# heyblackC/DFMIR

Measured on AMD Instinct MI355X. Metric: train-step image-pairs/sec (fwd+bwd): 2D 256x256 bs=16 and 3D 160^3 bs=1, higher is better.
Workload: dtype f32 (fp16x2-split MFMA, fp32 accumulate)

## Files before the change

### dfmir_amd/_lib.py

```python
import ctypes
import os
from ctypes import c_float, c_int, c_longlong, c_void_p, POINTER, Structure

_HERE = os.path.dirname(os.path.abspath(__file__))
LIB_PATH = os.environ.get("DFMIR_HIP_LIB") or os.path.join(_HERE, "libdfmir_hip.so")


class DfConvGeom(Structure):
    _fields_ = [(n, c_int) for n in (
        "N", "Cin", "Cout", "Di", "Hi", "Wi", "Do", "Ho", "Wo", "KD", "KH", "KW",
        "stride", "dil", "pd", "ph", "pw", "pad_mode", "act")] + [("slope", c_float)]


P = c_void_p
_GP = POINTER(DfConvGeom)
_SIGS = {
    "dfmir_abi_version": [],
    "dfmir_set_option": [ctypes.c_char_p, ctypes.c_char_p],
    "dfmir_get_option": [ctypes.c_char_p, ctypes.c_char_p, c_int],
    "dfmir_conv_fwd": [_GP, P, P, P, P, P],
    "dfmir_conv_wgrad": [_GP, P, P, P, P],
    "dfmir_bias_grad": [P, P, c_int, c_int, c_longlong, P],
    "dfmir_weight_pack": [P, P, c_int, c_int, c_int, c_int, P],
    "dfmir_weight_pack_floats": [c_int, c_int, c_int],
# ... 61 lines not shown
    "dfmir_instnorm_fwd": [P, P, P, P, P, c_int, c_longlong, c_float, c_int, P, P],
    "dfmir_instnorm_stats_ok": [c_longlong],
    "dfmir_instnorm_stats": [P, P, P, c_int, c_longlong, c_float, c_int, P, P],
    "dfmir_instnorm_bwd": [P, P, P, P, P, c_int, c_longlong, c_int, P, P],
    "dfmir_instnorm_bwd_cols_ok": [c_longlong, c_int],
    "dfmir_instnorm_bwd_cols": [P, P, P, P, P, c_int, c_longlong, c_int, P, P, c_int, P],
    "dfmir_in_relu_blurdown_ok": [c_int, c_int],
    "dfmir_in_relu_blurdown_fwd": [P, P, P, P, c_int, c_int, c_int, c_float, P, P],
    "dfmir_in_relu_blurdown_bwd": [P, P, P, P, P, c_int, c_int, c_int, P, P, P],
    "dfmir_act_bwd": [P, P, P, c_longlong, c_int, c_float, P],
    "dfmir_blur_down_fwd": [P, P, c_int, c_int, c_int, P],
    "dfmir_blur_down_bwd": [P, P, c_int, c_int, c_int, P],
    "dfmir_blur_up_fwd": [P, P, c_int, c_int, c_int, P],
    "dfmir_blur_up_bwd": [P, P, c_int, c_int, c_int, P],
    "dfmir_reflect_pad2d_fwd": [P, P, c_int, c_int, c_int, c_int, P],
    "dfmir_reflect_pad2d_bwd": [P, P, c_int, c_int, c_int, c_int, P],
    "dfmir_reflect_pad2d_bwd_add": [P, P, P, c_int, c_int, c_int, c_int, P],
    "dfmir_upcat_fwd": [P, P, P] + [c_int] * 7 + [P],
    "dfmir_upcat_bwd": [P, P, P] + [c_int] * 7 + [P],
    "dfmir_cat_channels_fwd": [P, P, P, c_longlong, c_longlong, c_longlong, P],
    "dfmir_cat_channels_bwd": [P, P, P, c_longlong, c_longlong, c_longlong, P],
    "dfmir_scale": [P, P, c_longlong, c_float, P],
    "dfmir_warp2d_fwd": [P, P, P] + [c_int] * 6 + [P],
    "dfmir_warp2d_bwd": [P, P, P, P, P] + [c_int] * 6 + [P],
    "dfmir_warp3d_fwd": [P, P, P] + [c_int] * 7 + [P],
    "dfmir_warp3d_bwd": [P, P, P, P, P] + [c_int] * 7 + [P],
    "dfmir_warp_bwd_own_ws_floats": [c_int] * 6,
    "dfmir_warp_bwd_own": [c_int, P, P, P, P, P] + [c_int] * 7 + [P, P],
    "dfmir_resize_fwd": [P, P] + [c_int] * 7 + [c_float, P],
    "dfmir_resize_bwd": [P, P] + [c_int] * 7 + [c_float, P],
    "dfmir_resize_bwd_ws_floats": [c_int] * 7,
    "dfmir_resize_bwd_sep": [P, P] + [c_int] * 7 + [c_float, P, P],
    "dfmir_patch_gather_fwd": [P, P, P, c_int, c_int, c_longlong, c_int, P],
    "dfmir_patch_gather_bwd": [P, P, P, c_int, c_int, c_longlong, c_int, P],
    "dfmir_patch_gather_bwd_amax": [P, P, P, c_int, c_int, c_longlong, c_int, P, P],
    "dfmir_patch_gather_fwd_g": [P, P, P, c_int, c_int, c_longlong, c_int, c_int, P],
    "dfmir_patch_gather_bwd_g": [P, P, P, c_int, c_int, c_longlong, c_int, c_int, P, P],
    "dfmir_l2norm_fwd": [P, P, P, c_int, c_longlong, c_float, P],
    "dfmir_l2norm_bwd": [P, P, P, P, c_int, c_longlong, c_float, P],
    "dfmir_patchnce_fwd": [P, P, P, P, c_longlong, c_int, c_int, c_float, P],
    "dfmir_patchnce_bwd": [P, P, P, P, c_longlong, c_int, c_int, c_float, P],
    "dfmir_masked_l1_fwd": [P, P, P, c_float, P, P, c_longlong, P],
    "dfmir_masked_l1_bwd": [P, P, P, c_float, P, P, P, P, c_longlong, P],
    "dfmir_flow_smooth_ws_floats": [],
    "dfmir_flow_smooth_fwd": [P, P, P] + [c_int] * 5 + [P],
    "dfmir_flow_smooth_bwd": [P, P, P] + [c_int] * 5 + [P],
    "dfmir_flow_smooth_fwd_p": [P, P, P] + [c_int] * 6 + [P],
    "dfmir_flow_smooth_bwd_p": [P, P, P] + [c_int] * 6 + [P],
    "dfmir_mul": [P, P, P, c_longlong, P],
    "dfmir_bend_ws_floats": [c_int] * 5,
    "dfmir_bend_fwd": [P, P, P] + [c_int] * 5 + [c_float] * 3 + [P],
    "dfmir_bend_bwd": [P, P, P] + [c_int] * 5 + [c_float] * 3 + [P],
    "dfmir_invcons_ws_floats": [c_int] * 5,
    "dfmir_invcons_fwd": [c_int, P, P, P, P, P, P] + [c_int] * 4 + [P],
    "dfmir_invcons_bwd_ws_floats": [c_int] * 5,
    "dfmir_invcons_bwd": [c_int, P, P, P, P, P, P, P] + [c_int] * 4 + [P],
    "dfmir_nmi_ws_floats": [c_longlong, c_int],
    "dfmir_nmi_fwd": [P, P, P, P, c_int, c_float, c_float, c_longlong, P, P, P],
    "dfmir_nmi_bwd": [P, P, P, P, c_int, c_float, c_float, c_longlong, P, P, P, P, P],
    "dfmir_mind_ws_floats": [c_int] * 8,
    "dfmir_mind_desc": [P] + [c_int] * 7 + [P, P, P],
    "dfmir_mind_fwd": [P, P, P] + [c_int] * 7 + [P, P, P],
    "dfmir_mind_bwd": [P, P, P] + [c_int] * 7 + [P, P, P, P, P, P],
    "dfmir_warp_dice_ws_floats": [c_int] * 6,
    "dfmir_warp_dice_fwd": [c_int, P, P, P, P] + [c_int] * 6 + [P, P, P, P, P],
    "dfmir_warp_dice_bwd": [c_int, P, P, P, P] + [c_int] * 5 + [P, P, P, P],
    "dfmir_label_hausdorff_ws_bytes": [c_int] * 6,
    "dfmir_label_edt_sq": [c_int, P, c_int, c_int] + [c_int] * 4 + [P, P],
    "dfmir_label_hausdorff": [c_int, P, P, P] + [c_int] * 7 + [P, P, P, P, P, P],
    "dfmir_dice_ws_floats": [c_longlong, c_longlong],
    "dfmir_dice_fwd": [P, P, c_longlong, c_longlong, P, P, P],
    "dfmir_dice_bwd": [P, P, c_longlong, c_longlong, P, P, P, P, P],
    "dfmir_mse_ws_floats": [c_longlong],
    "dfmir_mse_fwd": [P, P, c_longlong, P, P, P],
    "dfmir_mse_bwd": [P, P, c_longlong, P, P, P, P],
    "dfmir_ncc_fwd_m": [P, P, P, c_int, P, P, P, P] + [c_int] * 5 + [c_float, P],
    "dfmir_ncc_bwd_m": [P, P, P, c_int, P, P, P, P, P, P] + [c_int] * 5 + [c_float, P],
    "dfmir_ncc_gauss_fwd": [P, P, P, c_int, P, P, P, P] + [c_int] * 4 + [P, c_int, c_float, c_float, P],
    "dfmir_ncc_gauss_bwd": [P, P, P, c_int, P, P, P, P, P, P] + [c_int] * 4 + [P, c_int, c_float, c_float, P],
    "dfmir_ncc_fwd": [P, P, P, P, P, P] + [c_int] * 5 + [c_float, P],
    "dfmir_ncc_bwd": [P, P, P, P, P, P, P, P] + [c_int] * 5 + [c_float, P],
    "dfmir_patch_gather_fwd_multi": [P, c_int, P, P, c_int, c_int, c_longlong, c_int, P],
    "dfmir_nce_head_fwd": [P, c_int, P, P, P, P, P, P, P, P, P, P, c_int, c_int, c_longlong, c_int, c_float, P],
    "dfmir_patch_ids_draw": [P, P, c_int, c_int, c_int, P, P],
    "dfmir_segment_means_fwd": [P, P, c_int, c_int, c_longlong, c_float, P],
    "dfmir_segment_means_bwd": [P, P, c_int, c_int, c_longlong, c_float, P],
    "dfmir_scalar_combine_fwd": [P, c_int, P, c_int, P, P],
    "dfmir_scalar_combine_bwd": [P, c_int, P, c_int, P, P],
    "dfmir_det_head_floats": [],
    "dfmir_det_begin": [P, c_longlong, P, c_longlong, P, c_int, P, c_longlong, P, c_int, ctypes.c_double, P],
    "dfmir_det_end": [P, P, c_longlong, P, c_longlong, P],
    "dfmir_fill_zero": [P, c_longlong, P],
    "dfmir_sum_scaled": [P, P, c_longlong, c_float, P],
    "dfmir_fill_from_scalar": [P, P, c_longlong, c_float, P],
    "dfmir_adam_step": [P, P, P, P, c_longlong] + [c_float] * 7 + [P],
}

_lib = None


class DfmirHipError(RuntimeError):
    pass


def lib():
    global _lib
    if _lib is None:
        import torch
        if not os.path.exists(LIB_PATH):
            raise DfmirHipError(
                "libdfmir_hip.so not found at %s -- build it with `python -c 'import __graft_entry__ as g; "
                "g.build()'` or `make -C dfmir_amd/csrc` (there is no CPU fallback)" % LIB_PATH)
        h = ctypes.CDLL(LIB_PATH)
        for name, args in _SIGS.items():
            fn = getattr(h, name)
            fn.argtypes = args
            fn.restype = c_int
        h.dfmir_weight_pack_floats.restype = c_longlong
        h.dfmir_conv3d_split_ws_floats.restype = c_longlong
        h.dfmir_conv3d_up_ws_floats.restype = c_longlong
        h.dfmir_conv3d_up_dgrad_ws_floats.restype = c_longlong
        h.dfmir_conv3d_upwgrad_ws_floats.restype = c_longlong
        h.dfmir_flow_smooth_ws_floats.restype = c_longlong
        h.dfmir_bend_ws_floats.restype = c_longlong
        h.dfmir_invcons_ws_floats.restype = c_longlong
        h.dfmir_invcons_bwd_ws_floats.restype = c_longlong
        h.dfmir_nmi_ws_floats.restype = c_longlong
        h.dfmir_mind_ws_floats.restype = c_longlong
        h.dfmir_warp_dice_ws_floats.restype = c_longlong
        h.dfmir_label_hausdorff_ws_bytes.restype = c_longlong
        h.dfmir_dice_ws_floats.restype = c_longlong
        h.dfmir_mse_ws_floats.restype = c_longlong
        h.dfmir_warp_bwd_own_ws_floats.restype = c_longlong
        h.dfmir_resize_bwd_ws_floats.restype = c_longlong
        h.dfmir_last_error.argtypes = []
        h.dfmir_last_error.restype = ctypes.c_char_p
        _lib = h
    return _lib


def check(rc):
    if rc != 0:
        msg = lib().dfmir_last_error()
        raise DfmirHipError(msg.decode() if msg else "dfmir_hip error %d" % rc)


def set_option(name, value=None):
    check(lib().dfmir_set_option(name.encode(), None if value is None else str(value).encode()))


def get_option(name):
    buf = ctypes.create_string_buffer(256)
    n = lib().dfmir_get_option(name.encode(), buf, 256)
    return None if n < 0 else buf.value.decode()


def exported_symbols():
    return sorted(list(_SIGS.keys()) + ["dfmir_last_error"])
```

### dfmir_amd/csrc/nce_head.hip

```cpp
#include "common.h"

#define DF_IDS_MAXP 1024
#define DF_IDS_MAXPERM 4096
struct DfIdSizes {
  long long S[8];
};

__device__ __forceinline__ unsigned long long df_mix64(unsigned long long z) {
  z += 0x9E3779B97F4A7C15ull;
  z = (z ^ (z >> 30)) * 0xBF58476D1CE4E5B9ull;
  z = (z ^ (z >> 27)) * 0x94D049BB133111EBull;
  return z ^ (z >> 31);
}

__global__ __launch_bounds__(256) void patch_ids_draw_k(unsigned long long* __restrict__ state, DfIdSizes sizes,
                                                        int n_layers, int n_sets, int P, int Ppad,
                                                        long long* __restrict__ out) {
  __shared__ unsigned long long el[DF_IDS_MAXPERM];
  __shared__ unsigned char lost[DF_IDS_MAXP];
  __shared__ int pending;
  const int layer = blockIdx.x / n_sets, set = blockIdx.x - layer * n_sets;
  const unsigned long long S = (unsigned long long)sizes.S[layer];
  const unsigned long long seed = state[0], counter = state[1];
  const unsigned long long stream = df_mix64(seed ^ df_mix64(counter * 0x100000001B3ull + (unsigned long long)blockIdx.x));
// ... 203 lines not shown
    _Pragma("unroll") for (int u = 0; u < NH_KB; ++u) {                                           \
      const int kr = 2 * u + hi;                                                                  \
      const bool ok = kr < (KTOT_);                                                               \
      ca0[u] = ok ? wp[(long long)kr * NH_M] : 0.f;                                               \
      ca1[u] = ok ? wp[(long long)kr * NH_M + 32] : 0.f;                                          \
    }                                                                                             \
    for (int j = 0; j < nb; ++j) {                                                                \
      if (j + 1 < nb) {                                                                           \
        _Pragma("unroll") for (int u = 0; u < NH_KB; ++u) {                                       \
          const int kr = 2 * ((j + 1) * NH_KB + u) + hi;                                          \
          const bool ok = kr < (KTOT_);                                                           \
          na0[u] = ok ? wp[(long long)kr * NH_M] : 0.f;                                           \
          na1[u] = ok ? wp[(long long)kr * NH_M + 32] : 0.f;                                      \
        }                                                                                         \
      }                                                                                           \
      _Pragma("unroll") for (int u = 0; u < NH_KB; ++u) {                                         \
        const int kr = 2 * (j * NH_KB + u) + hi;                                                  \
        const float bv = (SRC_)[kr * NH_R + l31];                                                 \
        acc[0] = __builtin_amdgcn_mfma_f32_32x32x2f32(ca0[u], bv, acc[0], 0, 0, 0);               \
        acc[1] = __builtin_amdgcn_mfma_f32_32x32x2f32(ca1[u], bv, acc[1], 0, 0, 0);               \
      }                                                                                           \
      _Pragma("unroll") for (int u = 0; u < NH_KB; ++u) { ca0[u] = na0[u]; ca1[u] = na1[u]; }     \
    }                                                                                             \
  }
  NH_GEMM(k.w1, k.C, Xs)
#pragma unroll
  for (int i = 0; i < 2; ++i)
#pragma unroll
    for (int e = 0; e < 16; ++e) {
      const int m = m0 + 32 * i + (e >> 2) * 8 + hi * 4 + (e & 3);
      float v = acc[i][e] + k.b1[m];
      v = v > 0.f ? v : 0.f;
      Hs[m * NH_R + l31] = v;
      if (k.hs && r0 + l31 < k.rows) k.hs[(long long)m * k.rows + r0 + l31] = v;
      acc[i][e] = 0.f;
    }
  __syncthreads();
  NH_GEMM(k.w2, NH_M, Hs)
#undef NH_GEMM
  float ss = 0.f;
#pragma unroll
  for (int i = 0; i < 2; ++i)
#pragma unroll
    for (int e = 0; e < 16; ++e) {
      const int m = m0 + 32 * i + (e >> 2) * 8 + hi * 4 + (e & 3);
      acc[i][e] += k.b2[m];
      ss += acc[i][e] * acc[i][e];
    }
  ss += __shfl_xor(ss, 32);
  if (hi == 0) red[wid][l31] = ss;
  __syncthreads();
  const float nr = sqrtf((red[0][l31] + red[1][l31]) + (red[2][l31] + red[3][l31]));
  const float inv = 1.f / (nr + k.eps);
  const long long rr = r0 + l31;
  if (rr < k.rows) {
    if (k.nrm && wid == 0 && hi == 0) k.nrm[rr] = nr;
#pragma unroll
    for (int i = 0; i < 2; ++i)
#pragma unroll
      for (int e = 0; e < 16; ++e) {
        const int m = m0 + 32 * i + (e >> 2) * 8 + hi * 4 + (e & 3);
        k.out[(long long)m * k.rows + rr] = acc[i][e] * inv;
        if (k.ypre) k.ypre[(long long)m * k.rows + rr] = acc[i][e];
      }
  }
}
extern "C" int dfmir_nce_head_fwd(const float* const* srcs, int G, const long long* ids, const float* w1, const float* b1,
                                  const float* w2, const float* b2, float* out, float* nrm, float* xs, float* hs,
                                  float* ypre, int Bper, int C, long long S, int P, float eps, void* stream) {
  DF_ARG_CHECK(srcs && ids && w1 && b1 && w2 && b2 && out && G > 0 && G <= 8 && Bper > 0 && C > 0 && C <= NH_CMAX && S > 0 && P > 0);
  NceHeadP k{};
  for (int g = 0; g < G; ++g) {
    DF_ARG_CHECK(srcs[g] != nullptr);
    k.srcs.p[g] = srcs[g];
  }
  k.ids = ids; k.w1 = w1; k.b1 = b1; k.w2 = w2; k.b2 = b2;
  k.out = out; k.nrm = nrm; k.xs = xs; k.hs = hs; k.ypre = ypre;
  k.G = G; k.Bper = Bper; k.C = C; k.P = P; k.S = S; k.rows = (long long)G * Bper * P; k.eps = eps;
  nce_head_fwd_k<<<(unsigned)((k.rows + NH_R - 1) / NH_R), 256, 0, (hipStream_t)stream>>>(k);
  DF_LAUNCH_CHECK();
  return 0;
}

__global__ __launch_bounds__(256) void segment_means_k(const float* __restrict__ rows, float* __restrict__ out, int L,
                                                       int T, long long seg, float scale) {
  __shared__ float sm[17];
  const int t = blockIdx.x;
  float s = 0.f;
  for (int l = 0; l < L; ++l) {
    const float* r = rows + ((long long)l * T + t) * seg;
    for (long long i = threadIdx.x; i < seg; i += 256) s += r[i];
  }
  s = block_sum(s, sm);
  if (threadIdx.x == 0) out[t] = s * (scale / (float)seg);
}
__global__ void segment_means_bwd_k(const float* __restrict__ g, float* __restrict__ drows, int L, int T, long long seg,
                                    float scale) {
  const long long total = (long long)L * T * seg;
  for (long long i = (long long)blockIdx.x * blockDim.x + threadIdx.x; i < total;
       i += (long long)gridDim.x * blockDim.x) {
    const int t = (int)((i / seg) % T);
    drows[i] = g[t] * (scale / (float)seg);
  }
}
extern "C" int dfmir_segment_means_fwd(const float* rows, float* out, int L, int T, long long seg, float scale,
                                       void* stream) {
  DF_ARG_CHECK(rows && out && L > 0 && T > 0 && seg > 0);
  segment_means_k<<<(unsigned)T, 256, 0, (hipStream_t)stream>>>(rows, out, L, T, seg, scale);
  DF_LAUNCH_CHECK();
  return 0;
}
extern "C" int dfmir_segment_means_bwd(const float* gout, float* drows, int L, int T, long long seg, float scale,
                                       void* stream) {
  DF_ARG_CHECK(gout && drows && L > 0 && T > 0 && seg > 0);
  segment_means_bwd_k<<<df_grid((long long)L * T * seg, 256, 1024), 256, 0, (hipStream_t)stream>>>(gout, drows, L, T, seg,
                                                                                                scale);
  DF_LAUNCH_CHECK();
  return 0;
}

struct DfCombine {
  const float* in[8];
  float M[8][8];
};
__global__ void scalar_combine_k(DfCombine c, int n_in, int n_out, float* __restrict__ out) {
  const int j = threadIdx.x;
  if (j < n_out) {
    float s = 0.f;
    for (int i = 0; i < n_in; ++i) s += c.M[j][i] * c.in[i][0];
    out[j] = s;
  }
}
__global__ void scalar_combine_bwd_k(DfCombine c, const float* __restrict__ g, int n_in, int n_out,
                                     float* __restrict__ din) {
  const int i = threadIdx.x;
  if (i < n_in) {
    float s = 0.f;
    for (int j = 0; j < n_out; ++j) s += c.M[j][i] * g[j];
    din[i] = s;
  }
}
extern "C" int dfmir_scalar_combine_fwd(const float* const* in, int n_in, const float* M, int n_out, float* out,
                                        void* stream) {
  DF_ARG_CHECK(in && M && out && n_in > 0 && n_in <= 8 && n_out > 0 && n_out <= 8);
  DfCombine c{};
  for (int i = 0; i < n_in; ++i) {
    DF_ARG_CHECK(in[i] != nullptr);
    c.in[i] = in[i];
  }
  for (int j = 0; j < n_out; ++j)
    for (int i = 0; i < n_in; ++i) c.M[j][i] = M[j * n_in + i];
  scalar_combine_k<<<1, 64, 0, (hipStream_t)stream>>>(c, n_in, n_out, out);
  DF_LAUNCH_CHECK();
  return 0;
}
extern "C" int dfmir_scalar_combine_bwd(const float* gout, int n_in, const float* M, int n_out, float* din,
                                        void* stream) {
  DF_ARG_CHECK(gout && M && din && n_in > 0 && n_in <= 8 && n_out > 0 && n_out <= 8);
  DfCombine c{};
  for (int j = 0; j < n_out; ++j)
    for (int i = 0; i < n_in; ++i) c.M[j][i] = M[j * n_in + i];
  scalar_combine_bwd_k<<<1, 64, 0, (hipStream_t)stream>>>(c, gout, n_in, n_out, din);
  DF_LAUNCH_CHECK();
  return 0;
}

// ... 10 lines not shown
```

### dfmir_amd/ops.py

```python
import collections
import ctypes
import functools
import os

import numpy as np
import torch
from torch.autograd import Function
from torch.autograd.function import once_differentiable

from ._lib import DfConvGeom, DfmirHipError, check, lib

_VP = ctypes.c_void_p


def _p(t):
    return None if t is None else _VP(t.data_ptr())


def _st():
    return _VP(torch.cuda.current_stream().cuda_stream)


def _need(*ts):
    for t in ts:
# ... 1925 lines not shown
def _cuda_device(device):
    device = torch.device("cuda" if device is None else device)
    if device.type != "cuda":
        raise DfmirHipError("patch ids are drawn on the HIP device, not on %s" % device)
    return torch.device("cuda", torch.cuda.current_device() if device.index is None else device.index)


def seed_patch_ids(seed, device=None):
    device = _cuda_device(device)
    new = torch.tensor([int(seed) & 0x7FFFFFFFFFFFFFFF, 0, 0], dtype=torch.int64)
    st = _IDS_STATE.get(device)
    if st is None:
        st = _IDS_STATE[device] = new.to(device)
    else:
        st.copy_(new)
    return st


def draw_patch_ids(sizes, n_sets, P, device):
    device = _cuda_device(device)
    st = _IDS_STATE.get(device)
    if st is None:
        st = seed_patch_ids(torch.initial_seed(), device)
    L = len(sizes)
    out = torch.empty((L, n_sets, P), device=device, dtype=torch.int64)
    sz = (ctypes.c_longlong * L)(*[int(s) for s in sizes])
    check(lib().dfmir_patch_ids_draw(_p(st), sz, L, int(n_sets), int(P), _p(out), _st()))
    return mark_distinct(out)


def patch_gather_multi(srcs, ids):
    _need(*srcs)
    _need(ids)
    G = len(srcs)
    srcs = [_c(s) for s in srcs]
    Bper, C = srcs[0].shape[0], srcs[0].shape[1]
    S = srcs[0].numel() // (Bper * C)
    for s_ in srcs:
        if tuple(s_.shape) != tuple(srcs[0].shape):
            raise DfmirHipError("patch_gather_multi: sources differ in shape")
    ids = _c(ids.to(torch.int64))
    if ids.dim() != 2 or ids.shape[0] != G:
        raise DfmirHipError("patch_gather_multi: ids must be [G, P]")
    Pn = ids.shape[1]
    out = torch.empty((C, G * Bper * Pn), device=srcs[0].device, dtype=torch.float32)
    ptrs = (ctypes.c_void_p * G)(*[s_.data_ptr() for s_ in srcs])
    check(lib().dfmir_patch_gather_fwd_multi(ptrs, G, _p(ids), _p(out), Bper, C, S, Pn, _st()))
    return out


_NO_NCE_FUSED = _env_on("DFMIR_NO_NCE_FUSED")


def nce_head_ok(C, nc, use_mlp):
    return use_mlp and not _NO_NCE_FUSED and nc == 256 and 1 <= C <= 256


def _nce_head_launch(ptrs, G, ids, mlp0, mlp2, Bper, C, S, Pn, eps, device, save):
    rows = G * Bper * Pn
    out = torch.empty((256, rows), device=device, dtype=torch.float32)
    nrm = xs = hs = ypre = None
    if save:
        nrm = torch.empty(rows, device=device, dtype=torch.float32)
        xs = torch.empty((C, rows), device=device, dtype=torch.float32)
        hs = torch.empty((256, rows), device=device, dtype=torch.float32)
        ypre = torch.empty((256, rows), device=device, dtype=torch.float32)
    arr = (ctypes.c_void_p * G)(*ptrs)
    check(lib().dfmir_nce_head_fwd(arr, G, _p(ids), _p(mlp0.packed(0)), _p(mlp0.bias), _p(mlp2.packed(0)), _p(mlp2.bias),
                                   _p(out), _p(nrm), _p(xs), _p(hs), _p(ypre), Bper, C, S, Pn, float(eps), _st()))
    return out, nrm, xs, hs, ypre


def nce_head_multi(srcs, ids, mlp0, mlp2, eps=1e-7):
    _need(*srcs)
    srcs = [_c(s_) for s_ in srcs]
    Bper, C = srcs[0].shape[0], srcs[0].shape[1]
    S = srcs[0].numel() // (Bper * C)
    ids = _c(ids.to(torch.int64))
    out, _, _, _, _ = _nce_head_launch([s_.data_ptr() for s_ in srcs], len(srcs), ids, mlp0, mlp2, Bper, C, S, ids.shape[1], eps,
                                       srcs[0].device, False)
    return out


class NceHeadFn(Function):

    @staticmethod
    def forward(ctx, feat, ids, w1, b1, w2, b2, mlp0, mlp2, eps, distinct):
        _need(feat, ids)
        ctx.stash = getattr(feat, "_df_tap_stash", None) if feat.is_contiguous() else None
        feat = _c(feat)
        ids = _c(ids.to(torch.int64))
        G, Pn = ids.shape
        B, C = feat.shape[0], feat.shape[1]
        if B % G:
            raise DfmirHipError("nce_head: ids [G,P] with G dividing the batch")
        Bper = B // G
        S = feat.numel() // (B * C)
        base = feat.data_ptr()
        ptrs = [base + 4 * g * Bper * C * S for g in range(G)]
        out, nrm, xs, hs, ypre = _nce_head_launch(ptrs, G, ids, mlp0, mlp2, Bper, C, S, Pn, eps, feat.device, True)
        ctx.save_for_backward(ids, nrm, xs, hs, ypre, w1, w2)
        ctx.meta = (tuple(feat.shape), B, C, S, Pn, G, bool(distinct), float(eps))
        ctx.mods = (mlp0, mlp2)
        return out

    @staticmethod
    @once_differentiable
    def backward(ctx, dout):
        ids, nrm, xs, hs, ypre, w1, w2 = ctx.saved_tensors
        shape, B, C, S, Pn, G, distinct, eps = ctx.meta
        mlp0, mlp2 = ctx.mods
        rows = B * Pn
        dout = _c(dout)
        dy = torch.empty_like(ypre)
        check(lib().dfmir_l2norm_bwd(_p(dout), _p(ypre), _p(nrm), _p(dy), 256, rows, eps, _st()))
        c2 = _Ctx()
        c2.cfg, c2.x_amax, c2.dead_tail, c2.in_act, c2.has_bias = (2, (1, 1, 1), 1, (0, 0, 0), 0, 0, 0.0, mlp2), None, 0, None, True
        c2.needs_input_grad = (True, ctx.needs_input_grad[4], ctx.needs_input_grad[5])
        dh, dw2, db2 = _conv_backward_impl(c2, dy.view(1, 256, 1, rows), None, hs.view(1, 256, 1, 1, rows),
                                           w2.view(256, 256, 1, 1), None)
        c1 = _Ctx()
        c1.cfg, c1.x_amax, c1.dead_tail, c1.in_act, c1.has_bias = (2, (1, 1, 1), 1, (0, 0, 0), 0, 1, 0.0, mlp0), None, 0, None, True
        c1.needs_input_grad = (ctx.needs_input_grad[0], ctx.needs_input_grad[2], ctx.needs_input_grad[3])
        dx, dw1, db1 = _conv_backward_impl(c1, dh, None, xs.view(1, C, 1, 1, rows), w1.view(256, C, 1, 1),
                                           hs.view(1, 256, 1, 1, rows))
        dfeat = None
        if dx is not None:
            dxr = _c(dx).view(C, rows)
            meta = (shape, B, C, S, Pn, G, distinct)
            if ctx.stash is not None:
                ctx.stash.append((dxr, ids, meta))
            else:
                dfeat = zeros(shape, dxr.device)
                if distinct:
                    check(lib().dfmir_patch_gather_bwd_g(_p(dxr), _p(ids), _p(dfeat), B, C, S, Pn, G, None, _st()))
                else:
                    check(lib().dfmir_patch_gather_bwd_any(_p(dxr), _p(ids), _p(dfeat), B, C, S, Pn, G, None, None, _st()))
        dw1 = dw1.view(256, C) if dw1 is not None else None
        dw2 = dw2.view(256, 256) if dw2 is not None else None
        return dfeat, None, dw1, db1, dw2, db2, None, None, None, None


def nce_head(feat, ids, mlp0, mlp2, eps=1e-7):
    groups = ids.shape[0] if ids.dim() == 2 else 1
    ids2 = ids if ids.dim() == 2 else ids.view(1, -1)
    distinct = ids_distinct(ids, groups) if (torch.is_grad_enabled() and feat.requires_grad) else True
    return NceHeadFn.apply(feat, ids2, mlp0.weight, mlp0.bias, mlp2.weight, mlp2.bias, mlp0, mlp2, eps, distinct)


_LAST_L1_WS = [None]


class MaskedL1Fn(Function):
    @staticmethod
    def forward(ctx, a, b, mask, thr):
        _need(a, b, mask)
        a, b = _c(a), _c(b)
        m = None
        if mask is not None:
            m = _c(mask.to(torch.bool))
            if m.shape != a.shape:
                m = _c(m.expand_as(a))
        ws = torch.empty(8, device=a.device, dtype=torch.float32)
        out = torch.empty((), device=a.device, dtype=torch.float32)
        check(lib().dfmir_masked_l1_fwd(_p(a), _p(b), _p(m), float(thr), _p(ws), _p(out), a.numel(), _st()))
        _LAST_L1_WS[0] = ws
        ctx.save_for_backward(a, b, m, ws)
        ctx.thr = float(thr)
        return out

    @staticmethod
    @once_differentiable
    def backward(ctx, g):
        a, b, m, ws = ctx.saved_tensors
        g = _c(g)
        da = torch.empty_like(a) if ctx.needs_input_grad[0] else None
        db = torch.empty_like(b) if ctx.needs_input_grad[1] else None
        if da is not None or db is not None:
            check(lib().dfmir_masked_l1_bwd(_p(a), _p(b), _p(m), ctx.thr, _p(ws), _p(g), _p(da), _p(db),
                                            a.numel(), _st()))
        return da, db, None, None


def masked_l1(a, b, mask=None, thr=-0.95):
    out = MaskedL1Fn.apply(a, b, mask, thr)
    out._df_mask_sum = _LAST_L1_WS[0][1]
    return out


class FlowSmoothFn(Function):
    @staticmethod
    def forward(ctx, flow, penalty=2):
        _need(flow)
        flow = _c(flow)
        nd = flow.dim() - 2
        B, C = flow.shape[0], flow.shape[1]
        D, H, W = flow.shape[2:] if nd == 3 else (1,) + tuple(flow.shape[2:])
        ws = torch.empty(int(lib().dfmir_flow_smooth_ws_floats()), device=flow.device, dtype=torch.float32)
        out = torch.empty((), device=flow.device, dtype=torch.float32)
        if penalty == 2:
            check(lib().dfmir_flow_smooth_fwd(_p(flow), _p(ws), _p(out), B, C, D, H, W, _st()))
        else:
            check(lib().dfmir_flow_smooth_fwd_p(_p(flow), _p(ws), _p(out), B, C, D, H, W, int(penalty), _st()))
        ctx.save_for_backward(flow)
        ctx.meta = (B, C, D, H, W, int(penalty))
        return out

    @staticmethod
# ... 710 lines not shown
```

### include/dfmir_hip.h

```cpp
#ifndef DFMIR_HIP_H
#define DFMIR_HIP_H

#ifdef __cplusplus
extern "C" {
#endif

#define DFMIR_ABI_VERSION 14

int dfmir_abi_version(void);
const char* dfmir_last_error(void);

int dfmir_set_option(const char* name, const char* value);
int dfmir_get_option(const char* name, char* buf, int buf_len);

typedef struct DfConvGeom {
  int N, Cin, Cout;
  int Di, Hi, Wi;
  int Do, Ho, Wo;
  int KD, KH, KW;
  int stride, dil;
  int pd, ph, pw;
  int pad_mode;
  int act;
  float slope;
// ... 125 lines not shown
int dfmir_instnorm_fwd(const float* x, const float* res, float* y, float* mean, float* rstd,
                       int planes, long long S, float eps, int relu, float* y_amax, void* stream);
int dfmir_instnorm_bwd(const float* dy, const float* x, const float* mean, const float* rstd,
                       float* dx, int planes, long long S, int relu, float* dx_amax, void* stream);
int dfmir_instnorm_bwd_cols_ok(long long S, int W);
int dfmir_instnorm_bwd_cols(const float* dy, const float* x, const float* mean, const float* rstd, float* dx, int planes,
                            long long S, int relu, float* dx_amax, float* dx_cols, int W, void* stream);
int dfmir_instnorm_bwd_pmax_ok(long long S);
int dfmir_instnorm_bwd_pmax(const float* dy, const float* x, const float* mean, const float* rstd, float* dx, int planes,
                            long long S, int relu, float* dx_amax, float* dx_cols, int W, float* dx_pmax, void* stream);

int dfmir_in_relu_blurdown_ok(int H, int W);
int dfmir_in_relu_blurdown_fwd(const float* x, float* z, float* mean, float* rstd, int planes, int H, int W, float eps,
                               float* z_amax, void* stream);
int dfmir_in_relu_blurdown_bwd(const float* dz, const float* x, const float* mean, const float* rstd, float* dx,
                               int planes, int H, int W, float* dx_amax, float* dx_pmax, void* stream);

int dfmir_act_bwd(const float* dy, const float* y, float* dx, long long n, int act, float slope,
                  void* stream);
int dfmir_act_bwd_amax(const float* dy, const float* y, float* dx, long long n, int act, float slope,
                       float* dx_amax, void* stream);

int dfmir_blur_down_fwd(const float* x, float* y, int planes, int H, int W, void* stream);
int dfmir_blur_down_bwd(const float* dy, float* dx, int planes, int H, int W, void* stream);
int dfmir_blur_up_fwd(const float* x, float* y, int planes, int H, int W, void* stream);
int dfmir_blur_up_bwd(const float* dy, float* dx, int planes, int H, int W, void* stream);
int dfmir_reflect_pad2d_fwd(const float* x, float* y, int planes, int H, int W, int p, void* stream);
int dfmir_reflect_pad2d_bwd(const float* dy, float* dx, int planes, int H, int W, int p, void* stream);
int dfmir_reflect_pad2d_bwd_add(const float* dy, const float* add, float* dx, int planes, int H, int W, int p,
                                void* stream);

int dfmir_upcat_fwd(const float* a, const float* b, float* y, int N, int Ca, int Cb, int Da, int Ha,
                    int Wa, int sd, void* stream);
int dfmir_upcat_bwd(const float* dy, float* da, float* db, int N, int Ca, int Cb, int Da, int Ha,
                    int Wa, int sd, void* stream);

int dfmir_cat_channels_fwd(const float* a, const float* b, float* y, long long N, long long SA,
                           long long SB, void* stream);
int dfmir_cat_channels_bwd(const float* dy, float* da, float* db, long long N, long long SA,
                           long long SB, void* stream);
int dfmir_scale(const float* x, float* y, long long n, float mult, void* stream);

int dfmir_warp2d_fwd(const float* src, const float* flow, float* out, int B, int C, int H, int W,
                     int mode, int add_identity, void* stream);
int dfmir_warp2d_bwd(const float* dout, const float* src, const float* flow, float* dsrc,
                     float* dflow, int B, int C, int H, int W, int add_identity, int flow_into_src,
                     void* stream);
int dfmir_warp3d_fwd(const float* src, const float* flow, float* out, int B, int C, int D, int H,
                     int W, int mode, int add_identity, void* stream);
int dfmir_warp3d_bwd(const float* dout, const float* src, const float* flow, float* dsrc,
                     float* dflow, int B, int C, int D, int H, int W, int add_identity,
                     int flow_into_src, void* stream);
long long dfmir_warp_bwd_own_ws_floats(int nd, int B, int C, int D, int H, int W);
int dfmir_warp_bwd_own(int nd, const float* dout, const float* src, const float* flow, float* dsrc, float* dflow, int B,
                       int C, int D, int H, int W, int add_identity, int flow_into_src, float* ws, void* stream);

int dfmir_resize_fwd(const float* x, float* y, int planes, int Di, int Hi, int Wi, int Do, int Ho,
                     int Wo, float mult, void* stream);
int dfmir_resize_bwd(const float* dy, float* dx, int planes, int Di, int Hi, int Wi, int Do, int Ho,
                     int Wo, float mult, void* stream);
long long dfmir_resize_bwd_ws_floats(int planes, int Di, int Hi, int Wi, int Do, int Ho, int Wo);
int dfmir_resize_bwd_sep(const float* dy, float* dx, int planes, int Di, int Hi, int Wi, int Do, int Ho, int Wo,
                         float mult, float* ws, void* stream);

int dfmir_patch_gather_fwd(const float* feat, const long long* ids, float* out, int B, int C,
                           long long S, int P, void* stream);
int dfmir_patch_gather_bwd(const float* dout, const long long* ids, float* dfeat, int B, int C,
                           long long S, int P, void* stream);
int dfmir_patch_gather_bwd_amax(const float* dout, const long long* ids, float* dfeat, int B, int C, long long S,
                                int P, float* dfeat_amax, void* stream);
int dfmir_patch_gather_fwd_g(const float* feat, const long long* ids, float* out, int B, int C, long long S, int P,
                             int G, void* stream);
int dfmir_patch_gather_bwd_g(const float* dout, const long long* ids, float* dfeat, int B, int C, long long S, int P,
                             int G, float* dfeat_amax, void* stream);
int dfmir_patch_gather_bwd_gp(const float* dout, const long long* ids, float* dfeat, int B, int C, long long S, int P,
                              int G, float* dfeat_amax, float* dfeat_pmax, void* stream);
int dfmir_patch_gather_bwd_any(const float* dout, const long long* ids, float* dfeat, int B, int C, long long S, int P,
                               int G, float* dfeat_amax, float* dfeat_pmax, void* stream);
int dfmir_patch_gather_fwd_multi(const float* const* srcs, int G, const long long* ids, float* out, int Bper, int C,
                                 long long S, int P, void* stream);
int dfmir_nce_head_fwd(const float* const* srcs, int G, const long long* ids, const float* w1, const float* b1,
                       const float* w2, const float* b2, float* out, float* nrm, float* xs, float* hs, float* ypre,
                       int Bper, int C, long long S, int P, float eps, void* stream);
int dfmir_patch_ids_draw(unsigned long long* state, const long long* sizes, int n_layers, int n_sets, int P,
                         long long* out, void* stream);
int dfmir_l2norm_fwd(const float* x, float* y, float* norm, int C, long long rows, float eps, void* stream);
int dfmir_l2norm_bwd(const float* dy, const float* x, const float* norm, float* dx, int C,
                     long long rows, float eps, void* stream);
int dfmir_patchnce_fwd(const float* q, const float* k, float* loss, float* probs, long long rows,
                       int C, int G, float T, void* stream);
int dfmir_patchnce_bwd(const float* dloss, const float* probs, const float* k, float* dq,
                       long long rows, int C, int G, float T, void* stream);

int dfmir_masked_l1_fwd(const float* a, const float* b, const unsigned char* mask, float thr,
                        float* ws, float* out, long long n, void* stream);
int dfmir_masked_l1_bwd(const float* a, const float* b, const unsigned char* mask, float thr,
                        const float* ws, const float* gout, float* da, float* db, long long n,
                        void* stream);
long long dfmir_flow_smooth_ws_floats(void);
int dfmir_flow_smooth_fwd(const float* flow, float* ws, float* out, int B, int C, int D, int H,
                          int W, void* stream);
int dfmir_flow_smooth_bwd(const float* flow, const float* gout, float* dflow, int B, int C, int D,
                          int H, int W, void* stream);
int dfmir_flow_smooth_fwd_p(const float* flow, float* ws, float* out, int B, int C, int D, int H,
                            int W, int penalty, void* stream);
int dfmir_flow_smooth_bwd_p(const float* flow, const float* gout, float* dflow, int B, int C, int D,
                            int H, int W, int penalty, void* stream);
long long dfmir_bend_ws_floats(int B, int C, int D, int H, int W);
int dfmir_bend_fwd(const float* flow, float* ws, float* out, int B, int C, int D, int H, int W, float hz, float hy,
                   float hx, void* stream);
int dfmir_bend_bwd(const float* flow, const float* gout, float* dflow, int B, int C, int D, int H, int W, float hz,
                   float hy, float hx, void* stream);
long long dfmir_invcons_ws_floats(int nd, int B, int D, int H, int W);
int dfmir_invcons_fwd(int nd, const float* u, const float* v, float* ws, float* per_sample, float* loss, float* rmax, int B,
                      int D, int H, int W, void* stream);
long long dfmir_invcons_bwd_ws_floats(int nd, int B, int D, int H, int W);
int dfmir_invcons_bwd(int nd, const float* u, const float* v, const float* gout, const float* rmax, float* du, float* dv,
                      float* ws, int B, int D, int H, int W, void* stream);
long long dfmir_nmi_ws_floats(long long n, int nb);
int dfmir_nmi_fwd(const float* y_true, const float* y_pred, const float* mask, const float* centers, int nb,
                  float preterm, float max_clip, long long n, float* ws, float* out, void* stream);
int dfmir_nmi_bwd(const float* y_true, const float* y_pred, const float* mask, const float* centers, int nb,
                  float preterm, float max_clip, long long n, const float* ws, const float* gout, float* d_true,
                  float* d_pred, void* stream);
long long dfmir_mind_ws_floats(int nd, int B, int D, int H, int W, int radius, int dilation, int which);
int dfmir_mind_desc(const float* I, int nd, int B, int D, int H, int W, int radius, int dilation, float* ws, float* out,
                    void* stream);
int dfmir_mind_fwd(const float* a, const float* b, const float* mask, int nd, int B, int D, int H, int W, int radius,
                   int dilation, float* ws, float* out, void* stream);
int dfmir_mind_bwd(const float* a, const float* b, const float* mask, int nd, int B, int D, int H, int W, int radius,
                   int dilation, const float* ws, float* tmp, const float* gout, float* da, float* db, void* stream);
long long dfmir_warp_dice_ws_floats(int nd, int B, int K, int D, int H, int W);
int dfmir_warp_dice_fwd(int nd, const unsigned char* mov, const unsigned char* fix, const float* flow,
                        const unsigned char* slot_of, int K, int B, int D, int H, int W, int mode, float* ws,
                        float* loss, float* dice, float* seeds, void* stream);
int dfmir_warp_dice_bwd(int nd, const unsigned char* mov, const unsigned char* fix, const float* flow,
                        const unsigned char* slot_of, int K, int B, int D, int H, int W, const float* seeds,
                        const float* gout, float* dflow, void* stream);
#define DFMIR_EDT_SQ_INF (1 << 29)
#define DFMIR_HD_SURFACE 1
long long dfmir_label_hausdorff_ws_bytes(int nd, int B, int K, int D, int H, int W);
int dfmir_label_edt_sq(int nd, const unsigned char* map, int value, int surface, int B, int D, int H, int W, int* out,
                       void* stream);
int dfmir_label_hausdorff(int nd, const unsigned char* a, const unsigned char* b, const unsigned char* labels, int K, int B,
                          int D, int H, int W, int qm, int flags, void* ws, float* hd, float* directed, float* mean,
                          int* d2, void* stream);
long long dfmir_dice_ws_floats(long long planes, long long S);
int dfmir_dice_fwd(const float* y_true, const float* y_pred, long long planes, long long S, float* ws, float* out,
                   void* stream);
int dfmir_dice_bwd(const float* y_true, const float* y_pred, long long planes, long long S, const float* ws,
                   const float* gout, float* d_true, float* d_pred, void* stream);
long long dfmir_mse_ws_floats(long long n);
int dfmir_mse_fwd(const float* y_true, const float* y_pred, long long n, float* ws, float* out, void* stream);
int dfmir_mse_bwd(const float* y_true, const float* y_pred, long long n, const float* gout, float* d_true, float* d_pred,
                  void* stream);
int dfmir_mul(const float* a, const float* b, float* out, long long n, void* stream);
int dfmir_ncc_fwd(const float* I, const float* J, float* tmp, float* tmp2, float* ws, float* out,
                  int B, int D, int H, int W, int win, float eps, void* stream);
int dfmir_ncc_bwd(const float* I, const float* J, const float* sums, float* tmp, float* tmp2,
                  const float* ws, const float* gout, float* dI, int B, int D, int H, int W,
                  int win, float eps, void* stream);
#define DFMIR_NCC_VOLUME 4
int dfmir_ncc_fwd_m(const float* I, const float* J, const float* mask, int mode, float* tmp, float* tmp2,
                    float* ws, float* out, int B, int D, int H, int W, int win, float eps, void* stream);
int dfmir_ncc_bwd_m(const float* I, const float* J, const float* mask, int mode, const float* sums,
                    float* tmp, float* tmp2, const float* ws, const float* gout, float* dI, int B, int D,
// ... 28 lines not shown
```

Measured before the change: 219.9.

## Fuse NCE head backward into one data-grad kernel plus one batched wgrad kernel

Replaces the NCE projection-head backward (l2norm backward, then two generic 1x1 conv backward passes) with a fused kernel. It computes the normalisation gradient, the layer-2 data gradient with the ReLU mask, and the layer-1 data gradient in one pass, keeping intermediates in shared memory and using fp32 MFMA. A second kernel computes both layers' weight and bias gradients in one launch, accumulating atomically. The aim is to cut launch count and intermediate round trips for a small head, at the cost of a specialised path that is disabled under determinism, probe or profiler modes.

```diff
diff --git a/dfmir_amd/_lib.py b/dfmir_amd/_lib.py
--- a/dfmir_amd/_lib.py
+++ b/dfmir_amd/_lib.py
@@ -167,6 +167,9 @@
     "dfmir_ncc_bwd": [P, P, P, P, P, P, P, P] + [c_int] * 5 + [c_float, P],
     "dfmir_patch_gather_fwd_multi": [P, c_int, P, P, c_int, c_int, c_longlong, c_int, P],
     "dfmir_nce_head_fwd": [P, c_int, P, P, P, P, P, P, P, P, P, P, c_int, c_int, c_longlong, c_int, c_float, P],
+    "dfmir_nce_head_bwd_ok": [c_int],
+    "dfmir_nce_head_bwd": [P, P, P, P, P, P, P, P, P, c_int, c_longlong, c_float, P],
+    "dfmir_nce_head_wgrad": [P, P, P, P, P, P, P, P, c_int, c_longlong, P],
     "dfmir_patch_ids_draw": [P, P, c_int, c_int, c_int, P, P],
     "dfmir_segment_means_fwd": [P, P, c_int, c_int, c_longlong, c_float, P],
     "dfmir_segment_means_bwd": [P, P, c_int, c_int, c_longlong, c_float, P],
diff --git a/dfmir_amd/csrc/nce_head.hip b/dfmir_amd/csrc/nce_head.hip
--- a/dfmir_amd/csrc/nce_head.hip
+++ b/dfmir_amd/csrc/nce_head.hip
@@ -309,6 +309,258 @@
   return 0;
 }
 
+struct NceHeadBwdP {
+  const float *dout, *ypre, *nrm, *hs, *w2d, *w1d;
+  float *dy, *dh, *dx;
+  int C;
+  long long rows;
+  float eps;
+};
+constexpr int NH_BKB = 32;
+__device__ __forceinline__ void nh_bwd_gemm(const float* __restrict__ w, int ld, int mlim, int m0, int l31, int hi,
+                                            const float* src, nh_f32x16 (&acc)[2]) {
+  const float* wp = w + m0 + l31;
+  const bool ok0 = m0 + l31 < mlim, ok1 = m0 + 32 + l31 < mlim;
+  constexpr int nb = NH_M / 2 / NH_BKB;
+  float ca0[NH_BKB], ca1[NH_BKB], na0[NH_BKB], na1[NH_BKB];
+#pragma unroll
+  for (int u = 0; u < NH_BKB; ++u) {
+    const int kr = 2 * u + hi;
+    ca0[u] = ok0 ? wp[(long long)kr * ld] : 0.f;
+    ca1[u] = ok1 ? wp[(long long)kr * ld + 32] : 0.f;
+  }
+  for (int j = 0; j < nb; ++j) {
+    if (j + 1 < nb) {
+#pragma unroll
+      for (int u = 0; u < NH_BKB; ++u) {
+        const int kr = 2 * ((j + 1) * NH_BKB + u) + hi;
+        na0[u] = ok0 ? wp[(long long)kr * ld] : 0.f;
+        na1[u] = ok1 ? wp[(long long)kr * ld + 32] : 0.f;
+      }
+    }
+#pragma unroll
+    for (int u = 0; u < NH_BKB; ++u) {
+      const int kr = 2 * (j * NH_BKB + u) + hi;
+      const float bv = src[kr * NH_R + l31];
+      acc[0] = __builtin_amdgcn_mfma_f32_32x32x2f32(ca0[u], bv, acc[0], 0, 0, 0);
+      acc[1] = __builtin_amdgcn_mfma_f32_32x32x2f32(ca1[u], bv, acc[1], 0, 0, 0);
+    }
+#pragma unroll
+    for (int u = 0; u < NH_BKB; ++u) { ca0[u] = na0[u]; ca1[u] = na1[u]; }
+  }
+}
+__global__ __launch_bounds__(256, 2) void nce_head_bwd_k(NceHeadBwdP k) {
+  __shared__ float Ys[NH_M * NH_R];
+  __shared__ float Hs[NH_M * NH_R];
+  __shared__ float red[4][NH_R];
+  const int tid = threadIdx.x, lane = tid & 63, wid = tid >> 6;
+  const int l31 = lane & 31, hi = lane >> 5;
+  const int m0 = 64 * wid;
+  const long long rr = (long long)blockIdx.x * NH_R + l31;
+  const bool rok = rr < k.rows;
+  nh_f32x16 acc[2];
+  unsigned relu = 0u;
+  {
+    float dv[2][16], yv[2][16], hv[2][16];
+    float dot = 0.f;
+#pragma unroll
+    for (int i = 0; i < 2; ++i)
+#pragma unroll
+      for (int e = 0; e < 16; ++e) {
+        const int m = m0 + 32 * i + (e >> 2) * 8 + hi * 4 + (e & 3);
+        dv[i][e] = rok ? k.dout[(long long)m * k.rows + rr] : 0.f;
+        yv[i][e] = rok ? k.ypre[(long long)m * k.rows + rr] : 0.f;
+        hv[i][e] = rok ? k.hs[(long long)m * k.rows + rr] : 0.f;
+      }
+#pragma unroll
+    for (int i = 0; i < 2; ++i)
+#pragma unroll
+      for (int e = 0; e < 16; ++e) relu |= (hv[i][e] > 0.f ? 1u : 0u) << (16 * i + e);
+#pragma unroll
+    for (int i = 0; i < 2; ++i)
+#pragma unroll
+      for (int e = 0; e < 16; ++e) dot += dv[i][e] * yv[i][e];
+    dot += __shfl_xor(dot, 32);
+    if (hi == 0) red[wid][l31] = dot;
+    __syncthreads();
+    dot = (red[0][l31] + red[1][l31]) + (red[2][l31] + red[3][l31]);
+    const float n = rok ? k.nrm[rr] : 0.f;
+    const float inv = 1.f / (n + k.eps);
+    const float k2 = n > 0.f ? dot * inv * inv / n : 0.f;
+#pragma unroll
+    for (int i = 0; i < 2; ++i)
+#pragma unroll
+      for (int e = 0; e < 16; ++e) {
+        const int m = m0 + 32 * i + (e >> 2) * 8 + hi * 4 + (e & 3);
+        const float v = rok ? dv[i][e] * inv - yv[i][e] * k2 : 0.f;
+        Ys[m * NH_R + l31] = v;
+        if (rok) k.dy[(long long)m * k.rows + rr] = v;
+        acc[i][e] = 0.f;
+      }
+  }
+  __syncthreads();
+  {
+    nh_bwd_gemm(k.w2d, NH_M, NH_M, m0, l31, hi, Ys, acc);
+#pragma unroll
+    for (int i = 0; i < 2; ++i)
+#pragma unroll
+      for (int e = 0; e < 16; ++e) {
+        const int m = m0 + 32 * i + (e >> 2) * 8 + hi * 4 + (e & 3);
+        const float v = ((relu >> (16 * i + e)) & 1u) ? acc[i][e] : 0.f;
+        Hs[m * NH_R + l31] = v;
+        if (rok) k.dh[(long long)m * k.rows + rr] = v;
+        acc[i][e] = 0.f;
+      }
+  }
+  if (!k.dx) return;
+  __syncthreads();
+  if (m0 >= k.C) return;
+  nh_bwd_gemm(k.w1d, k.C, k.C, m0, l31, hi, Hs, acc);
+  if (rok) {
+#pragma unroll
+    for (int i = 0; i < 2; ++i)
+#pragma unroll
+      for (int e = 0; e < 16; ++e) {
+        const int m = m0 + 32 * i + (e >> 2) * 8 + hi * 4 + (e & 3);
+        if (m < k.C) k.dx[(long long)m * k.rows + rr] = acc[i][e];
+      }
+  }
+}
+
+struct NceHeadWgradP {
+  const float *x0, *x1, *d0, *d1;
+  float *dw0, *dw1, *db0, *db1;
+  int C;
+  long long rows, chunks, chunks_per_block;
+};
+template <bool V4>
+__global__ __launch_bounds__(256, 2) void nce_head_wgrad_k(NceHeadWgradP k) {
+  constexpr int BK = 64, LD = BK + 1;
+  __shared__ float Xs[64 * LD];
+  __shared__ float Ds[64 * LD];
+  const int tid = threadIdx.x, lane = tid & 63, wid = tid >> 6;
+  const int l31 = lane & 31, lhi = lane >> 5, wm = wid >> 1, wn = wid & 1;
+  const int prob = blockIdx.z >> 2;
+  const int Cin = prob ? k.C : NH_M;
+  const int ci0 = blockIdx.y * 64, co0 = (blockIdx.z & 3) * 64;
+  if (ci0 >= Cin) return;
+  const float* __restrict__ x = prob ? k.x1 : k.x0;
+  const float* __restrict__ dy = prob ? k.d1 : k.d0;
+  float* __restrict__ dwt = prob ? k.dw1 : k.dw0;
+  float* __restrict__ db = ci0 == 0 ? (prob ? k.db1 : k.db0) : nullptr;
+  const long long S = k.rows;
+  const long long cbeg = (long long)blockIdx.x * k.chunks_per_block;
+  long long cend = cbeg + k.chunks_per_block;
+  if (cend > k.chunks) cend = k.chunks;
+  const int r = tid >> 2, q16 = (tid & 3) * 16;
+  const bool xrow = ci0 + r < Cin;
+  const float* xp = x + (long long)(ci0 + r) * S + q16;
+  const float* dp = dy + (long long)(co0 + r) * S + q16;
+  float4 rx[4], rd[4];
+  const float4 z4 = make_float4(0.f, 0.f, 0.f, 0.f);
+  float bsum = 0.f;
+  auto gload = [&](long long c) {
+    const long long q0 = c * BK;
+#pragma unroll
+    for (int j = 0; j < 4; ++j) {
+      const long long q = q0 + q16 + 4 * j;
+      if (V4) {
+        const bool in = q < S;
+        const float4 vx = *reinterpret_cast<const float4*>((xrow && in) ? xp + q0 + 4 * j : x);
+        const float4 vd = *reinterpret_cast<const float4*>(in ? dp + q0 + 4 * j : dy);
+        rx[j] = (xrow && in) ? vx : z4;
+        rd[j] = in ? vd : z4;
+      } else {
+        const float* a = xp + q0 + 4 * j;
+        const float* b = dp + q0 + 4 * j;
+        rx[j].x = (xrow && q < S) ? a[0] : 0.f;
+        rx[j].y = (xrow && q + 1 < S) ? a[1] : 0.f;
+        rx[j].z = (xrow && q + 2 < S) ? a[2] : 0.f;
+        rx[j].w = (xrow && q + 3 < S) ? a[3] : 0.f;
+        rd[j].x = q < S ? b[0] : 0.f;
+        rd[j].y = q + 1 < S ? b[1] : 0.f;
+        rd[j].z = q + 2 < S ? b[2] : 0.f;
+        rd[j].w = q + 3 < S ? b[3] : 0.f;
+      }
+    }
+  };
+  auto lstore = [&]() {
+    float* xs_ = &Xs[r * LD + q16];
+    float* ds_ = &Ds[r * LD + q16];
+#pragma unroll
+    for (int j = 0; j < 4; ++j) {
+      xs_[4 * j] = rx[j].x; xs_[4 * j + 1] = rx[j].y; xs_[4 * j + 2] = rx[j].z; xs_[4 * j + 3] = rx[j].w;
+      ds_[4 * j] = rd[j].x; ds_[4 * j + 1] = rd[j].y; ds_[4 * j + 2] = rd[j].z; ds_[4 * j + 3] = rd[j].w;
+      bsum += (rd[j].x + rd[j].y) + (rd[j].z + rd[j].w);
+    }
+  };
+  nh_f32x16 acc;
+#pragma unroll
+  for (int i = 0; i < 16; ++i) acc[i] = 0.f;
+  if (cbeg < cend) gload(cbeg);
+  for (long long c = cbeg; c < cend; ++c) {
+    __syncthreads();
+    lstore();
+    __syncthreads();
+    if (c + 1 < cend) gload(c + 1);
+    const float* ap = &Xs[(wm * 32 + l31) * LD + lhi];
+    const float* bp = &Ds[(wn * 32 + l31) * LD + lhi];
+#pragma unroll 8
+    for (int ks = 0; ks < BK / 2; ++ks)
+      acc = __builtin_amdgcn_mfma_f32_32x32x2f32(ap[2 * ks], bp[2 * ks], acc, 0, 0, 0);
+  }
+  if (cbeg >= cend) return;
+  const int co = co0 + wn * 32 + l31;
+#pragma unroll
+  for (int i = 0; i < 16; ++i) {
+    const int ci = ci0 + wm * 32 + 4 * lhi + (i & 3) + 8 * (i >> 2);
+    if (ci < Cin) df_acc(dwt, (long long)ci * NH_M + co, acc[i], nullptr);
+  }
+  if (db) {
+    bsum += __shfl_xor(bsum, 1);
+    bsum += __shfl_xor(bsum, 2);
+    if ((tid & 3) == 0) df_acc(db, co0 + r, bsum, nullptr);
+  }
+}
+
+extern "C" int dfmir_nce_head_bwd_ok(int C) {
+  static DfOptFlag off_o{"DFMIR_NO_NCE_BWD_FUSED"};
+  return (C >= 1 && C <= NH_CMAX && !off_o.get()) ? 1 : 0;
+}
+extern "C" int dfmir_nce_head_bwd(const float* dout, const float* ypre, const float* nrm, const float* hs, const float* w2d,
+                                  const float* w1d, float* dy, float* dh, float* dx, int C, long long rows, float eps,
+                                  void* stream) {
+  DF_ARG_CHECK(dout && ypre && nrm && hs && w2d && w1d && dy && dh && C > 0 && C <= NH_CMAX && rows > 0 &&
+               rows < (1LL << 31) * NH_R);
+  NceHeadBwdP k{};
+  k.dout = dout; k.ypre = ypre; k.nrm = nrm; k.hs = hs; k.w2d = w2d; k.w1d = w1d;
+  k.dy = dy; k.dh = dh; k.dx = dx; k.C = C; k.rows = rows; k.eps = eps;
+  nce_head_bwd_k<<<(unsigned)((rows + NH_R - 1) / NH_R), 256, 0, (hipStream_t)stream>>>(k);
+  DF_LAUNCH_CHECK();
+  return 0;
+}
+extern "C" int dfmir_nce_head_wgrad(const float* xs, const float* hs, const float* dy, const float* dh, float* dw1,
+                                    float* db1, float* dw2, float* db2, int C, long long rows, void* stream) {
+  DF_ARG_CHECK(xs && hs && dy && dh && dw1 && db1 && dw2 && db2 && C > 0 && C <= NH_CMAX && rows > 0);
+  NceHeadWgradP k{};
+  k.x0 = hs; k.d0 = dy; k.dw0 = dw2; k.db0 = db2;
+  k.x1 = xs; k.d1 = dh; k.dw1 = dw1; k.db1 = db1;
+  k.C = C; k.rows = rows;
+  k.chunks = (rows + 63) / 64;
+  long long want = 1024 / 16;
+  long long maxs = (k.chunks + 7) / 8;
+  if (want > maxs) want = maxs;
+  k.chunks_per_block = (k.chunks + want - 1) / want;
+  const unsigned nx = (unsigned)((k.chunks + k.chunks_per_block - 1) / k.chunks_per_block);
+  const dim3 grid(nx, NH_M / 64, 2 * (NH_M / 64));
+  const bool v4 = (rows & 3) == 0 && ((reinterpret_cast<uintptr_t>(xs) | reinterpret_cast<uintptr_t>(hs) |
+                                      reinterpret_cast<uintptr_t>(dy) | reinterpret_cast<uintptr_t>(dh)) & 15) == 0;
+  if (v4) nce_head_wgrad_k<true><<<grid, 256, 0, (hipStream_t)stream>>>(k);
+  else nce_head_wgrad_k<false><<<grid, 256, 0, (hipStream_t)stream>>>(k);
+  DF_LAUNCH_CHECK();
+  return 0;
+}
+
 __global__ __launch_bounds__(256) void segment_means_k(const float* __restrict__ rows, float* __restrict__ out, int L,
                                                        int T, long long seg, float scale) {
   __shared__ float sm[17];
diff --git a/dfmir_amd/ops.py b/dfmir_amd/ops.py
--- a/dfmir_amd/ops.py
+++ b/dfmir_amd/ops.py
@@ -2031,6 +2031,42 @@
     return out
 
 
+_LAST_NCE_BWD_FUSED = [False]
+
+
+def last_nce_bwd_fused():
+    return _LAST_NCE_BWD_FUSED[0]
+
+
+def _nce_bwd_fused_ok(C, needs):
+    if _DET["on"] or _PROBE_AUDIT["on"] or _CONV_PROFILER[0] is not None or not all(needs[2:6]):
+        return False
+    return bool(lib().dfmir_nce_head_bwd_ok(int(C)))
+
+
+def _nce_grad_targets(owner, Cin, device):
+    defer = (_DEFER["on"] and owner.weight.grad is not None and owner.weight.grad.is_contiguous())
+    dwt = _deferred_buffer(owner, 1, Cin, 256, (256, Cin, 1, 1), device) if defer else zeros((1, Cin, 256), device)
+    bg = owner.bias.grad if defer else None
+    if bg is not None and bg.is_contiguous():
+        return dwt, bg, defer, True
+    return dwt, zeros(256, device), defer, False
+
+
+def _nce_head_backward_fused(dout, nrm, xs, hs, ypre, mlp0, mlp2, C, rows, eps, want_dx):
+    dev = dout.device
+    dy, dh = torch.empty_like(ypre), torch.empty_like(hs)
+    dx = torch.empty((C, rows), device=dev, dtype=torch.float32) if want_dx else None
+    check(lib().dfmir_nce_head_bwd(_p(dout), _p(ypre), _p(nrm), _p(hs), _p(mlp2.packed(1)), _p(mlp0.packed(1)),
+                                   _p(dy), _p(dh), _p(dx), C, rows, float(eps), _st()))
+    dwt1, db1, defer1, db1_in_place = _nce_grad_targets(mlp0, C, dev)
+    dwt2, db2, defer2, db2_in_place = _nce_grad_targets(mlp2, 256, dev)
+    check(lib().dfmir_nce_head_wgrad(_p(xs), _p(hs), _p(dy), _p(dh), _p(dwt1), _p(db1), _p(dwt2), _p(db2), C, rows, _st()))
+    dw1 = None if defer1 else weight_unpack(dwt1, (256, C, 1, 1)).view(256, C)
+    dw2 = None if defer2 else weight_unpack(dwt2, (256, 256, 1, 1)).view(256, 256)
+    return dx, dw1, None if db1_in_place else db1, dw2, None if db2_in_place else db2
+
+
 class NceHeadFn(Function):
 
     @staticmethod
@@ -2061,18 +2097,23 @@
         mlp0, mlp2 = ctx.mods
         rows = B * Pn
         dout = _c(dout)
-        dy = torch.empty_like(ypre)
-        check(lib().dfmir_l2norm_bwd(_p(dout), _p(ypre), _p(nrm), _p(dy), 256, rows, eps, _st()))
-        c2 = _Ctx()
-        c2.cfg, c2.x_amax, c2.dead_tail, c2.in_act, c2.has_bias = (2, (1, 1, 1), 1, (0, 0, 0), 0, 0, 0.0, mlp2), None, 0, None, True
-        c2.needs_input_grad = (True, ctx.needs_input_grad[4], ctx.needs_input_grad[5])
-        dh, dw2, db2 = _conv_backward_impl(c2, dy.view(1, 256, 1, rows), None, hs.view(1, 256, 1, 1, rows),
-                                           w2.view(256, 256, 1, 1), None)
-        c1 = _Ctx()
-        c1.cfg, c1.x_amax, c1.dead_tail, c1.in_act, c1.has_bias = (2, (1, 1, 1), 1, (0, 0, 0), 0, 1, 0.0, mlp0), None, 0, None, True
-        c1.needs_input_grad = (ctx.needs_input_grad[0], ctx.needs_input_grad[2], ctx.needs_input_grad[3])
-        dx, dw1, db1 = _conv_backward_impl(c1, dh, None, xs.view(1, C, 1, 1, rows), w1.view(256, C, 1, 1),
-                                           hs.view(1, 256, 1, 1, rows))
+        _LAST_NCE_BWD_FUSED[0] = _nce_bwd_fused_ok(C, ctx.needs_input_grad)
+        if _LAST_NCE_BWD_FUSED[0]:
+            dx, dw1, db1, dw2, db2 = _nce_head_backward_fused(dout, nrm, xs, hs, ypre, mlp0, mlp2, C, rows, eps,
+                                                              ctx.needs_input_grad[0])
+        else:
+            dy = torch.empty_like(ypre)
+            check(lib().dfmir_l2norm_bwd(_p(dout), _p(ypre), _p(nrm), _p(dy), 256, rows, eps, _st()))
+            c2 = _Ctx()
+            c2.cfg, c2.x_amax, c2.dead_tail, c2.in_act, c2.has_bias = (2, (1, 1, 1), 1, (0, 0, 0), 0, 0, 0.0, mlp2), None, 0, None, True
+            c2.needs_input_grad = (True, ctx.needs_input_grad[4], ctx.needs_input_grad[5])
+            dh, dw2, db2 = _conv_backward_impl(c2, dy.view(1, 256, 1, rows), None, hs.view(1, 256, 1, 1, rows),
+                                               w2.view(256, 256, 1, 1), None)
+            c1 = _Ctx()
+            c1.cfg, c1.x_amax, c1.dead_tail, c1.in_act, c1.has_bias = (2, (1, 1, 1), 1, (0, 0, 0), 0, 1, 0.0, mlp0), None, 0, None, True
+            c1.needs_input_grad = (ctx.needs_input_grad[0], ctx.needs_input_grad[2], ctx.needs_input_grad[3])
+            dx, dw1, db1 = _conv_backward_impl(c1, dh, None, xs.view(1, C, 1, 1, rows), w1.view(256, C, 1, 1),
+                                               hs.view(1, 256, 1, 1, rows))
         dfeat = None
         if dx is not None:
             dxr = _c(dx).view(C, rows)
diff --git a/include/dfmir_hip.h b/include/dfmir_hip.h
--- a/include/dfmir_hip.h
+++ b/include/dfmir_hip.h
@@ -231,6 +231,11 @@
 int dfmir_nce_head_fwd(const float* const* srcs, int G, const long long* ids, const float* w1, const float* b1,
                        const float* w2, const float* b2, float* out, float* nrm, float* xs, float* hs, float* ypre,
                        int Bper, int C, long long S, int P, float eps, void* stream);
+int dfmir_nce_head_bwd_ok(int C);
+int dfmir_nce_head_bwd(const float* dout, const float* ypre, const float* nrm, const float* hs, const float* w2d,
+                       const float* w1d, float* dy, float* dh, float* dx, int C, long long rows, float eps, void* stream);
+int dfmir_nce_head_wgrad(const float* xs, const float* hs, const float* dy, const float* dh, float* dw1, float* db1,
+                         float* dw2, float* db2, int C, long long rows, void* stream);
 int dfmir_patch_ids_draw(unsigned long long* state, const long long* sizes, int n_layers, int n_sets, int P,
                          long long* out, void* stream);
 int dfmir_l2norm_fwd(const float* x, float* y, float* norm, int C, long long rows, float eps, void* stream);
```

Result: no change. 221.1, median of 6 (+0.5%).
